# BUTSpeechFIT/huggingface_asr

Hardware: AMD Instinct MI355X
Metric: audio-seconds/sec encoder fwd+CTC, E-Branchformer-base (higher is better)
Workload: dtype bf16; 1 GPU; E-Branchformer-base enc+CTC (relative-pos), 32x10s 16kHz clips/GPU: fbank+CMVN -> conv2d sub -> 16 layers -> CTC head -> CTC loss (the batch-independent projection of the relative-position table, 0.2 % of the FLOPs, is cached across steps); per_gpu_batch=32, frames=1000, encoder_frames=250, parallelism=replicas x1 (no exchange step), steps_in_flight=4, wide_tiles=True, hw_queues=4

## Files before the change

### huggingface_asr_amd/_lib.py

```python
from __future__ import annotations

import ctypes as C
import os

_HERE = os.path.dirname(os.path.abspath(__file__))
LIB_PATH = os.environ.get("HFASR_HIP_LIB") or os.path.join(_HERE, "libhfasr_hip.so")

vp, i32, i64, f32, f64, sz = C.c_void_p, C.c_int, C.c_long, C.c_float, C.c_double, C.c_size_t


class EbfConfig(C.Structure):
    _fields_ = [(n, i32) for n in ("B", "T", "F", "d", "H", "I", "L", "V", "C1", "C2", "K", "stride", "pad",
                                   "is_causal", "pos_type", "csgu_kernel", "merge_kernel", "csgu_act", "use_macaron")] + \
               [("ln_eps", f32), ("logits_f32", i32), ("logits_ld", i32), ("branch_overlap", i32), ("extra_layers", i32), ("layer_mixing", i32), ("csgu_linear", i32),
                ("context_mode", i32), ("gate_blk", i32), ("ln_fold", i32), ("wide_tiles", i32)]


class LnRedDesc(C.Structure):
    _fields_ = [("partial", vp), ("nblk", i32), ("d", i32), ("dgamma", vp), ("dbeta", vp), ("kind", i32)]


class Gpt2Config(C.Structure):
    _fields_ = [("d", i32), ("H", i32), ("L", i32), ("V", i32), ("eps", f32), ("step_form", i32), ("act", i32)]

# ... 20 lines not shown
    "mi_layernorm_chain": [vp, i64, vp, i32, vp, vp, f32, vp, i64, vp, vp, f32, vp, i64, vp, i64, vp, vp, vp, i64, i32, i32, vp],
    "mi_cast_f32_bf16": [vp, i64, vp, i64, i32, i32, vp],
    "mi_rotary_bf16": [vp, i64, vp, i64, vp, vp, i32, i32, i32, i32, vp],
    "mi_attention_bf16": [vp, i64, vp, i64, vp, i64, i32, vp, i64, vp, vp, vp, vp, i64, i32, i32, i32, i32, f32, i32, vp],
    "mi_attention_qkv_bf16": [vp, i64, vp, i64, vp, i64, vp, i64, vp, vp, vp, vp, i64, i32, i32, i32, i64, i32, i32, f32, i32, vp],
    "mi_attention_qkv_bf16_v": [vp, i64, vp, i64, vp, i64, vp, i64, vp, vp, vp, vp, i64, i32, i32, i32, i64, i32, i32, f32, i32, i32, vp],
    "mi_attention_x_lse_bf16": [vp, i64, vp, i64, vp, i64, vp, vp, i64, vp, i32, i32, i32, i32, i32, f32, i32, f32, C.c_uint, C.c_uint, vp],
    "mi_attention_x_bwd_probs": [vp, i64, vp, i64, vp, i64, vp, vp, i64, vp, i64, vp, vp, vp, i64, vp, i64, i32, i32, i32, i32, i32, f32, i32, f32, C.c_uint, C.c_uint, vp],
    "mi_attention_qkv_lse_bf16": [vp, i64, vp, i64, vp, i64, vp, i64, vp, vp, vp, vp, i64, vp, i32, i32, i32, i32, f32, i32, f32, C.c_uint, C.c_uint, vp],
    "mi_attention_qkv_bwd_probs": [vp, i64, vp, i64, vp, i64, vp, i64, vp, vp, vp, vp, i64, vp, i64, vp, vp, vp, i64, vp, i64, i32,
                                   vp, i64, vp, vp, vp, vp, i64, i32, i32, i32, i32, f32, i32, f32, C.c_uint, C.c_uint, i32, vp],
    "mi_attention_qkv_bwd_fused": [vp, vp, vp, i64, vp, vp, i64, vp, i64, vp, vp, vp, vp, i64, vp, sz, i32, i32, i32, i32, f32, vp],
    "mi_row_stats_bf16": [vp, i64, i32, f32, vp, i32, vp],
    "mi_csgu_bf16": [vp, i64, vp, vp, vp, vp, vp, vp, i64, i32, i32, i32, i32, i32, i32, i32, vp],
    "mi_dwconv_residual_bf16": [vp, i64, vp, vp, vp, i64, i32, i32, i32, i32, i32, vp],
    "mi_fbank_f64": [vp, i64, vp, i32, vp, vp, vp, vp, vp, vp, i32, i32, i32, f64, f64, vp],
    "mi_trim_zeros_pad_f32": [vp, i64, vp, i32, i32, i32, vp, i64, i32, vp, vp, vp, vp],
    "mi_cmvn_utterance": [vp, vp, i32, i32, i32, i32, i32, f32, vp],
    "mi_cmvn_global": [vp, i64, i32, vp, vp, vp],
    "mi_row_lse": [vp, i64, i32, i32, vp, i32, vp],
    "mi_gemm_lse_f32": [vp, i64, vp, i64, vp, vp, i64, vp, vp, i32, i32, i32, vp],
    "mi_gemm_lse_workspace_floats": [i32, i32],
    "mi_row_argmax": [vp, i64, i32, i32, vp, i32, vp],
    "mi_ctc_collapse": [vp, i32, i32, vp, i32, i64, vp, i32, vp, vp, vp],
    "mi_ctc_greedy": [vp, i64, i64, i32, i32, i32, i32, vp, i32, i64, vp, vp, i32, vp, vp, vp],
    "mi_ctc_beam_workspace_bytes": [i32, i32, i32],
    "mi_ctc_beam_cut": [vp, i64, i64, i32, i32, i32, i32, vp, i32, i32, vp, vp, vp, vp, vp],
    "mi_ctc_beam_walk": [vp, i64, i64, i32, i32, i32, i32, vp, i32, i64, i32, i32, i32, vp, vp, vp, vp, vp, sz, vp, i32, vp, vp, vp, vp],
    "mi_gemm_argmax_workspace_floats": [i32, i32],
    "mi_gemm_argmax_bf16": [vp, i64, vp, i64, vp, vp, vp, i32, i32, i32, vp],
# ... 167 lines not shown
```

### huggingface_asr_amd/csrc/encoder.hip

```cpp
#include "common.hpp"
#include <hip/hip_ext.h>
#include <stdio.h>
#include "../../include/hfasr_hip.h"

namespace {

enum G { G_CONV1_W, G_CONV1_B, G_CONV2_W, G_CONV2_B, G_FEOUT_W, G_FEOUT_B, G_FP_LN_G, G_FP_LN_B, G_FP_W, G_FP_B,
         G_ENC_LN_G, G_ENC_LN_B, G_HEAD_W, G_HEAD_B, G_MIX_W ,
         G_GATE1_W, G_GATE1_B, G_GATE2_W, G_GATE2_B  };
enum LS { FF1_LN_G, FF1_LN_B, FF1_W1, FF1_B1, FF1_W2, FF1_B2,
          ATT_LN_G, ATT_LN_B, ATT_WQK, ATT_BQK, ATT_WV, ATT_BV, ATT_WO, ATT_BO, ATT_WPOS, ATT_U, ATT_V,
          MLP_LN_G, MLP_LN_B, MLP_W1, MLP_B1, CSGU_LN_G, CSGU_LN_B, CSGU_W, CSGU_B, MLP_W2, MLP_B2,
          MRG_DW_W, MRG_DW_B, MRG_W, MRG_B, FIN_LN_G, FIN_LN_B,
          FF2_LN_G, FF2_LN_B, FF2_W1, FF2_B1, FF2_W2, FF2_B2, CSGU_LIN_W, CSGU_LIN_B,
          FF1_WF, FF1_SF, FF1_CF, QKV_WF, QKV_SF, QKV_CF, MLP_WF, MLP_SF, MLP_CF, FF2_WF, FF2_SF, FF2_CF };

struct Dims { int T1, F1, T2, F2, M, Tp, hd; };

int conv_out(int n, int k, int s, int pad_total) { return (n + pad_total - k) / s + 1; }

Dims dims(const mi_ebf_config& c) {
    Dims d;
    const int pt = c.is_causal ? 2 * c.pad : 2 * c.pad;
    d.T1 = conv_out(c.T, c.K, c.stride, pt); d.F1 = conv_out(c.F, c.K, c.stride, pt);
// ... 261 lines not shown
    if (!c.ln_fold) RUN(enter_layer(w.x, 0));
    if (c.layer_mixing) RUN(mi_softmax_vec_f32(Gf(G_MIX_W), c.L + 1, w.sw, st));
    const int P = 2 * T2 - 1;
    if (c.pos_type == 1 && compute_posp)
        for (int l = 0; l < Lt; ++l)
            RUN(mi_gemm_bf16(pos_table, d, Lw(l, ATT_WPOS), d, nullptr, 0, (bf16_t*)posp + (size_t)l * P * d, d, 0, nullptr, 0, 1.f, 0,
                             P, d, d, 0, 0, st));
    const float* rot_cos = (const float*)pos_table;
    const float* rot_sin = rot_cos ? rot_cos + (size_t)T2 * D.hd : nullptr;
    const float scale = 1.0f / sqrtf((float)D.hd);
    const int kc = c.csgu_kernel, km = c.merge_kernel;

    if (c.ln_fold) {
        if (c.pos_type == 2 || !c.use_macaron || c.extra_layers || c.layer_mixing || c.csgu_linear || (D.hd != 64 && D.hd != 128)) return MI_ERR_ARG;
        const int gv = c.wide_tiles ? 40 : 0;
        const int npg = c.wide_tiles ? d / 64 : d / 32;
        RUN(mi_layernorm_fold(w.x, d, mask_len, T2, nullptr, nullptr, 0.f, w.x, d, w.a0, d, w.lnst, M, d, st));
        int np = 1;
        for (int l = 0; l < c.L; ++l) {
            if (hidden_states && hipMemcpyAsync(hidden_states + (size_t)l * M * d, w.x, (size_t)M * d * sizeof(float), hipMemcpyDeviceToDevice, st) != hipSuccess)
                return MI_ERR_LAUNCH;
            RUN(mi_gemm_lnfold_bf16(w.a0, d, Lw(l, FF1_WF), d, Lf(l, FF1_SF), Lf(l, FF1_CF), w.lnst, np, leps, w.h, I, 1, M, I, d, st));
            RUN(mi_gemm_resid_stats_f32_v(w.h, I, Lw(l, FF1_W2), I, Lf(l, FF1_B2), w.x, d, w.x, d, 0.5f, w.a0, d, w.lnst, M, d, I, gv, st));
            np = npg;
            RUN(mi_gemm_lnfold_bf16(w.a0, d, Lw(l, QKV_WF), d, Lf(l, QKV_SF), Lf(l, QKV_CF), w.lnst, np, leps, w.qk, 3 * d, 0, M, 3 * d, d, st));
            RUN(mi_attention_qkv_bf16(w.qk, 3 * d, w.qk + d, 3 * d, w.qk + 2 * d, 3 * d,
                                      c.pos_type == 1 ? (const bf16_t*)posp + (size_t)l * P * d : nullptr, d,
                                      c.pos_type == 1 ? Lf(l, ATT_U) : nullptr, c.pos_type == 1 ? Lf(l, ATT_V) : nullptr,
                                      mask_len, w.ctx, d, c.B, T2, 0, 0, c.H, D.hd, scale, c.is_causal, st));
            RUN(mi_gemm_bf16_v(w.ctx, d, Lw(l, ATT_WO), d, Lf(l, ATT_BO), 1, w.cat, 2 * d, 0, nullptr, 0, 1.f, 0, M, d, d, 0, 0, gv, st));
            RUN(mi_gemm_lnfold_bf16(w.a0, d, Lw(l, MLP_WF), d, Lf(l, MLP_SF), Lf(l, MLP_CF), w.lnst, np, leps, w.h, I, 1, M, I, d, st));
            RUN(mi_row_stats_bf16(w.h + I / 2, I, I / 2, leps, w.stats, M, st));
            const int dil = c.is_causal ? (kc - 1) / 2 : 1;
            const int cpad = c.is_causal ? (kc - 1) * dil : (kc - 1) / 2;
            RUN(mi_csgu_bf16(w.h, I, w.stats, Lf(l, CSGU_LN_G), Lf(l, CSGU_LN_B), Lf(l, CSGU_W), Lf(l, CSGU_B), w.s, I / 2, c.B, T2, I / 2, kc, cpad, dil, c.csgu_act, st));
            RUN(mi_gemm_bf16_v(w.s, I / 2, Lw(l, MLP_W2), I / 2, Lf(l, MLP_B2), 1, w.cat + d, 2 * d, 0, nullptr, 0, 1.f, 0, M, d, I / 2, 0, 0, gv, st));
            RUN(mi_dwconv_residual_bf16(w.cat, 2 * d, Lf(l, MRG_DW_W), Lf(l, MRG_DW_B), w.m2, 2 * d, c.B, T2, 2 * d, km, (km - 1) / 2, st));
            RUN(mi_gemm_resid_stats_f32_v(w.m2, 2 * d, Lw(l, MRG_W), 2 * d, Lf(l, MRG_B), w.x, d, w.x, d, 1.0f, w.a0, d, w.lnst, M, d, 2 * d, gv, st));
            RUN(mi_gemm_lnfold_bf16(w.a0, d, Lw(l, FF2_WF), d, Lf(l, FF2_SF), Lf(l, FF2_CF), w.lnst, np, leps, w.h, I, 1, M, I, d, st));
            RUN(mi_gemm_bf16_v(w.h, I, Lw(l, FF2_W2), I, Lf(l, FF2_B2), 1, w.x, d, 1, w.x, d, 0.5f, 0, M, d, I, 0, 0, gv, st));
            if (l + 1 == c.L) {
                RUN(mi_layernorm_chain(w.x, d, nullptr, T2, Lf(l, FIN_LN_G), Lf(l, FIN_LN_B), leps, nullptr, 0,
                                       Gf(G_ENC_LN_G), Gf(G_ENC_LN_B), c.ln_eps, w.hid, d, last_hidden, d, nullptr, nullptr, nullptr, 0, M, d, st));
            } else {
                RUN(mi_layernorm_fold(w.x, d, nullptr, T2, Lf(l, FIN_LN_G), Lf(l, FIN_LN_B), leps, w.x, d, w.a0, d, w.lnst, M, d, st));
                np = 1;
            }
        }
    } else
    for (int l = 0; l < Lt; ++l) {
        if (hidden_states && l < c.L && hipMemcpyAsync(hidden_states + (size_t)l * M * d, w.x, (size_t)M * d * sizeof(float), hipMemcpyDeviceToDevice, st) != hipSuccess)
            return MI_ERR_LAUNCH;
// ... 144 lines not shown
```

### huggingface_asr_amd/csrc/gemm_8p.hip

```cpp
#include "gemm_args.hpp"
#include <type_traits>

#ifndef GEMM_FLOOR
#define GEMM_FLOOR 0
#endif
#ifndef GEMM128_LOADER
#define GEMM128_LOADER 0
#endif

namespace {

typedef __attribute__((address_space(1))) const void* gptr_t;
typedef __attribute__((address_space(3))) void* lptr_t;

constexpr int TB = 256, BK = 64;
constexpr int BUF = 65536, BOFF = 32768;

template <int N>
__device__ __forceinline__ void wait_vm() {
    if constexpr (N >= 0) asm volatile("s_waitcnt vmcnt(%0)" ::"n"(N) : "memory");
}
__device__ __forceinline__ void barrier() {
    __builtin_amdgcn_sched_barrier(0);
    asm volatile("s_barrier" ::: "memory");
    __builtin_amdgcn_sched_barrier(0);
}
__device__ __forceinline__ void wait_lds() {
    asm volatile("s_waitcnt lgkmcnt(0)" ::: "memory");
    __builtin_amdgcn_sched_barrier(0);
}

__device__ __attribute__((aligned(16))) uint4 g_zero_page8p = {0u, 0u, 0u, 0u};

struct Ctx {
    const char* A; const char* W;
    unsigned offA[2][2], offB[2][2];
    int cti[2][2], cfi[2][2];
    unsigned dA[2][2], dB[2][2];
    unsigned aRd[2], bRd[2];
};

template <bool CONV, int ACT, bool OUT32 = false, bool GATED = false, bool LNF = false, bool LSE = false, bool AMAX = false, int CE = 0>
__global__ __launch_bounds__(512, 2) void gemm8p_kernel(GemmArgs p) {
    extern __shared__ __attribute__((aligned(16))) char smem[];
    const int tid = threadIdx.x, lane = tid & 63;
    const int wave = __builtin_amdgcn_readfirstlane(tid >> 6);
    const int wr = wave >> 2, wc = wave & 3;

    const int ntm = (p.M + TB - 1) / TB, ntn = (p.N + TB - 1) / TB;
    const int nwg = ntm * ntn;
    int bid = blockIdx.x;
    {
        const int q = nwg >> 3, r = nwg & 7, xcd = bid & 7, idx = bid >> 3;
        bid = (xcd < r ? xcd * (q + 1) : r * (q + 1) + (xcd - r) * q) + idx;
    }
    const int m0 = (bid / ntn) * TB, n0 = (bid % ntn) * TB;

    Ctx c;
    c.A = reinterpret_cast<const char*>(p.A);
    c.W = reinterpret_cast<const char*>(p.W);
    {
        const int prow = lane >> 3, pc = lane & 7;
#pragma unroll
        for (int h = 0; h < 2; ++h)
#pragma unroll
            for (int e = 0; e < 2; ++e) {
                const int ra = wr * 128 + h * 64 + (2 * wc + e) * 8;
                const int rb = (wave >> 1) * 64 + h * 32 + (2 * (wave & 1) + e) * 8;
                const int lcA = pc ^ (((ra + prow) >> 1) & 7), lcB = pc ^ (((rb + prow) >> 1) & 7);
                if constexpr (CONV) {
                    const int m = min(m0 + ra + prow, p.M - 1);
// ... 151 lines not shown
    if (wr == 1) barrier();
    unsigned cb = 0;
    int kt = 0;
    for (; kt < nk - 2; ++kt) {
        tile(kt, cb, T{}, T{}, T{}, T{}, std::integral_constant<int, 8>{}, std::integral_constant<int, 8>{}, std::integral_constant<int, 8>{});
        cb ^= BUF;
    }
    tile(kt, cb, T{}, T{}, F{}, F{}, std::integral_constant<int, 8>{}, std::integral_constant<int, 8>{}, std::integral_constant<int, 4>{});
    cb ^= BUF;
    tile(kt + 1, cb, F{}, F{}, F{}, F{}, std::integral_constant<int, 2>{}, std::integral_constant<int, 0>{}, std::integral_constant<int, -1>{});
    if (wr == 0) barrier();

    char* reg = smem + wave * 16384;
    const int fr = lane & 15, fq = lane >> 4, swz = (fr >> 1) & 7;
    const int nb = n0 + wc * 64;
    if constexpr (OUT32) {
        const int n4 = (p.N + 3) & ~3;
        float* C = reinterpret_cast<float*>(p.C);
#pragma unroll
        for (int j = 0; j < 4; ++j) {
            const int n = nb + j * 16 + fq * 4;
            f32x4 bj = f32x4{0.f, 0.f, 0.f, 0.f};
            if (p.bias_mode == 1) {
#pragma unroll
                for (int e = 0; e < 4; ++e)
                    if (n + e < p.N) bj[e] = p.bias[n + e];
            }
#pragma unroll
            for (int i = 0; i < 8; ++i) acc[i][j] += bj;
        }
// ... 832 lines not shown
        if ((a.N % TB) != 0 || (a.ldc % 8) != 0) return false;
        if (a.bias_mode == 1 && ((uintptr_t)a.bias & 15)) return false;
    }
    if (a.gated && (!conv || a.out_f32 || a.act != 1)) return false;
    if (a.ln_stats) {
        if (conv || a.out_f32 || a.gated || a.act > 1 || a.bias_mode != 1 || !a.ln_colsum || ((uintptr_t)a.ln_colsum & 15) || ((uintptr_t)a.ln_stats & 15)) return false;
        if (!(a.ln_npart == 1 || (a.ln_npart >= 4 && a.ln_npart <= 16 && (a.ln_npart % 4) == 0))) return false;
    }
    if (a.act >= 3) {
        if (conv || a.out_f32 || a.gated || a.ln_stats || a.resid || a.col_T || a.act > 4 || (a.aux_kind != 1 && a.aux_kind != 2) || a.drop_p < 0.f || a.drop_p >= 1.f) return false;
        if (a.act == 3 && (!a.aux || ((uintptr_t)a.aux & 15) || (a.ldaux % 8))) return false;
        if (a.act == 4 && (!a.C2 || ((uintptr_t)a.C2 & 15) || (a.ldc2 % 8))) return false;
    } else if (a.C2 || a.stats_out) {
        if (!a.out_f32 || !a.resid || a.N > 1024 || (a.C2 && (((uintptr_t)a.C2 & 7) || (a.ldc2 % 4))) || ((uintptr_t)a.stats_out & 7)) return false;
    }
    if (a.lse_part && (conv || !a.out_f32 || a.resid || a.C2 || a.stats_out || a.act != 0 || ((uintptr_t)a.lse_part & 7) || (a.lse_ld % 2) || a.lse_ld < 8 * cdiv(a.N, TB))) return false;
    if (a.amax_part && (conv || !a.out_f32 || a.resid || a.C2 || a.stats_out || a.lse_part || a.act != 0 || ((uintptr_t)a.amax_part & 7) || (a.amax_ld % 2) || a.amax_ld < 8 * cdiv(a.N, TB))) return false;
    if (a.ce) {
        if (a.ce < 1 || a.ce > 2 || conv || !a.out_f32 || a.resid || a.C2 || a.stats_out || a.amax_part || a.act != 0 || !a.ce_labels) return false;
        if (a.ce == 1 && (!a.lse_part || !a.ce_target)) return false;
        if (a.ce == 2 && (a.lse_part || !a.C || !a.ce_lse || !a.ce_g || (a.ldc % 8) != 0 || a.ldc < a.N || a.ldc > (long)TB * cdiv(a.N, TB))) return false;
    }
    if ((long)a.N * a.ldw * 2 >= (1l << 32)) return false;
    if (conv) {
        if ((a.Cin % BK) != 0 || a.Fout <= 0 || a.Tout <= 0) return false;
        if ((long)cdiv(a.M, (long)a.Fout * a.Tout) * a.Tin * a.Fin * a.Cin * 2 >= (1l << 32)) return false;
    } else if ((a.lda % 8) || (long)a.M * a.lda * 2 >= (1l << 32)) return false;
    return true;
}

template <typename K>
static bool set_lds_attr(K kernel, int bytes) { return ensure_dynamic_lds_ptr(reinterpret_cast<const void*>(kernel), (size_t)bytes); }

int gemm_8p_launch(const GemmArgs& a, bool conv, hipStream_t stream) {
    using kern_t = void (*)(GemmArgs);
    static const kern_t kerns[2][3] = {{gemm8p_kernel<false, 0>, gemm8p_kernel<false, 1>, gemm8p_kernel<false, 2>},
                                       {gemm8p_kernel<true, 0>, gemm8p_kernel<true, 1>, gemm8p_kernel<true, 2>}};
    if (a.act >= 0 && a.act <= 2 && !set_lds_attr(kerns[conv ? 1 : 0][a.act], 2 * BUF)) return MI_ERR_LAUNCH;
    if (a.act < 0 || a.act > 4) return MI_ERR_ARG;
    const int grid = cdiv(a.M, TB) * cdiv(a.N, TB);
    if (a.act >= 3) {
        const bool attr_t = set_lds_attr(gemm8p_kernel<false, 3>, 2 * BUF) && set_lds_attr(gemm8p_kernel<false, 4>, 2 * BUF);
        (void)attr_t;
        if (a.act == 3) launch_dense(PF_8P, gemm8p_kernel<false, 3>, dim3(grid), dim3(512), (size_t)2 * BUF, stream, a);
        else launch_dense(PF_8P_GELU, gemm8p_kernel<false, 4>, dim3(grid), dim3(512), (size_t)2 * BUF, stream, a);
        return MI_OK;
    }
    if (a.out_f32 && a.ce) {
        const kern_t kc = a.ce == 1 ? gemm8p_kernel<false, 0, true, false, false, false, false, 1> : gemm8p_kernel<false, 0, true, false, false, false, false, 2>;
        if (!set_lds_attr(kc, 2 * BUF)) return MI_ERR_LAUNCH;
// ... 73 lines not shown
```

### huggingface_asr_amd/csrc/gemm_args.hpp

```cpp
#pragma once
#include "common.hpp"
#include <hip/hip_ext.h>

struct GemmArgs {
    const bf16_t* A; long lda;
    const bf16_t* W; long ldw;
    const float* bias; int bias_mode;
    void* C; long ldc; int out_f32;
    const float* resid; long ldr; float alpha;
    int act;
    int col_T, col_Tp;
    int M, N, K;
    int variant;
    int Tin, Fin, Cin, Tout, Fout, KW, stride, pad_t, pad_f;
    int stride_f;
    int gated;
    const float* ln_stats; int ln_npart; const float* ln_colsum; float ln_eps;
    bf16_t* C2; long ldc2; float* stats_out;
    const bf16_t* aux; long ldaux; int aux_kind; float drop_p; unsigned long long drop_key;
    float* lse_part; int lse_ld;
    float* amax_part; int amax_ld;
    int ce; const long* ce_labels; float* ce_target; const float* ce_lse; const float* ce_g;
};
constexpr int LN_STATS_STRIDE = 32;

bool gemm_glds_supported(const GemmArgs& a, bool conv);
int gemm_glds_launch(const GemmArgs& a, bool conv, hipStream_t stream);


bool gemm_8p_supported(const GemmArgs& a, bool conv);
int gemm_8p_launch(const GemmArgs& a, bool conv, hipStream_t stream);
bool gemm_8p128_supported(const GemmArgs& a);
int gemm_8p128_launch(const GemmArgs& a, int ring, hipStream_t stream);


extern "C" int mi_profile_take_events(hipEvent_t* start, hipEvent_t* stop, int family);
enum { PF_8P = 0, PF_8P_GELU = 1, PF_8P_CONV = 2, PF_8P_OUT32 = 3, PF_8P128 = 4, PF_GLDS = 5, PF_GENERIC = 6, PF_8P_AMAX = 7, PF_8P_CE = 8, PF_COUNT = 9 };
// ... 8 lines not shown
```

### huggingface_asr_amd/csrc/gemm_bf16.hip

```cpp
#include "gemm_args.hpp"

namespace {

constexpr int BM = 128, BN = 128, BK = 64;
constexpr int NT = 256;

__device__ __forceinline__ int swz(int row, int chunk) { return chunk ^ ((row >> 1) & 7); }

template <bool CONV>
__global__ __launch_bounds__(NT) void gemm_bf16_kernel(GemmArgs p) {
    extern __shared__ __attribute__((aligned(16))) char smem[];
    bf16_t* sA = reinterpret_cast<bf16_t*>(smem);
    bf16_t* sB = sA + 2 * BM * BK;

    const int tid = threadIdx.x;
    const int lane = tid & 63, wave = tid >> 6;
    const int wm = wave >> 1, wn = wave & 1;

    const int ntm = (p.M + BM - 1) / BM, ntn = (p.N + BN - 1) / BN;
    const int nwg = ntm * ntn;
    int bid = blockIdx.x;
    {
        const int q = nwg >> 3, r = nwg & 7, xcd = bid & 7, idx = bid >> 3;
        bid = (xcd < r ? xcd * (q + 1) : r * (q + 1) + (xcd - r) * q) + idx;
// ... 301 lines not shown
    GemmArgs a{};
    a.A = (const bf16_t*)A; a.lda = lda; a.W = (const bf16_t*)W; a.ldw = ldw; a.bias = bias; a.bias_mode = bias ? 1 : 0;
    a.C = C; a.ldc = ldc; a.out_f32 = 1; a.resid = resid; a.ldr = ldr; a.alpha = alpha; a.act = 0; a.M = M; a.N = N; a.K = K;
    a.C2 = (bf16_t*)C2; a.ldc2 = ldc2; a.stats_out = stats_out;
    if (!A || !W || !C || !resid || (variant != 0 && variant != 40 && variant != 42 && variant != 43)) return MI_ERR_ARG;
    const bool wide = variant == 40;
    if (wide ? !gemm_8p_supported(a, false) : !gemm_8p128_supported(a)) return MI_ERR_UNSUPPORTED;
    const int slot = mi_profile_hook_begin(stream, 2.0 * M * N * K);
    const int rc = wide ? gemm_8p_launch(a, false, stream) : gemm_8p128_launch(a, variant == 42 ? 3 : (variant == 43 ? 2 : 0), stream);
    if (slot >= 0) mi_profile_hook_end(slot, stream);
    if (rc != MI_OK) return rc;
    MI_CHECK_LAUNCH();
    return MI_OK;
}

namespace {
__global__ __launch_bounds__(256) void lse_merge_kernel(const float* __restrict__ part, int ld, int npair, float* __restrict__ lse, int M) {
    const int g = threadIdx.x & 15;
    const int row = blockIdx.x * 16 + (threadIdx.x >> 4);
    const float* pr = part + (long)min(row, M - 1) * ld;
    float mx = -INFINITY;
    for (int t = g; t < npair; t += 16) mx = fmaxf(mx, pr[2 * t]);
    mx = fmaxf(mx, dpp_f32<0xB1, 0xF>(mx, mx)); mx = fmaxf(mx, dpp_f32<0x4E, 0xF>(mx, mx));
    mx = fmaxf(mx, dpp_f32<0x141, 0xF>(mx, mx)); mx = fmaxf(mx, dpp_f32<0x140, 0xF>(mx, mx));
    float s = 0.f;
    for (int t = g; t < npair; t += 16) {
        const f32x2 q = *reinterpret_cast<const f32x2*>(pr + 2 * t);
        if (q.x > -INFINITY) s += q.y * __expf(q.x - mx);
    }
    s += dpp_f32<0xB1, 0xF>(0.f, s); s += dpp_f32<0x4E, 0xF>(0.f, s);
// ... 137 lines not shown
```

### huggingface_asr_amd/engine.py

```python
from __future__ import annotations

import ctypes as C
import os

import torch

from . import _lib, ops
from .packing import _enc_map, encoder_specs, mapped_fp32, packed, relative_position_table, rotary_tables
from .shapes import GATE_SHARE, context_mode

G = dict(CONV1_W=0, CONV1_B=1, CONV2_W=2, CONV2_B=3, FEOUT_W=4, FEOUT_B=5, FP_LN_G=6, FP_LN_B=7, FP_W=8, FP_B=9,
         ENC_LN_G=10, ENC_LN_B=11, HEAD_W=12, HEAD_B=13, MIX_W=14, GATE1_W=15, GATE1_B=16, GATE2_W=17, GATE2_B=18)
LS = {n: i for i, n in enumerate(
    ["FF1_LN_G", "FF1_LN_B", "FF1_W1", "FF1_B1", "FF1_W2", "FF1_B2",
     "ATT_LN_G", "ATT_LN_B", "ATT_WQK", "ATT_BQK", "ATT_WV", "ATT_BV", "ATT_WO", "ATT_BO", "ATT_WPOS", "ATT_U", "ATT_V",
     "MLP_LN_G", "MLP_LN_B", "MLP_W1", "MLP_B1", "CSGU_LN_G", "CSGU_LN_B", "CSGU_W", "CSGU_B", "MLP_W2", "MLP_B2",
     "MRG_DW_W", "MRG_DW_B", "MRG_W", "MRG_B", "FIN_LN_G", "FIN_LN_B",
     "FF2_LN_G", "FF2_LN_B", "FF2_W1", "FF2_B1", "FF2_W2", "FF2_B2", "CSGU_LIN_W", "CSGU_LIN_B",
     "FF1_WF", "FF1_SF", "FF1_CF", "QKV_WF", "QKV_SF", "QKV_CF", "MLP_WF", "MLP_SF", "MLP_CF", "FF2_WF", "FF2_SF", "FF2_CF"])}
SLOT_RENAME = {"att_wqkv": "ATT_WQK", "att_bqkv": "ATT_BQK"}
FOLDS = {"ff1_b1": ("FF1", "ff1_w1", "ff1_ln_g", "ff1_ln_b"), "att_bqkv": ("QKV", "att_wqkv", "att_ln_g", "att_ln_b"),
         "mlp_b1": ("MLP", "mlp_w1", "mlp_ln_g", "mlp_ln_b"), "ff2_b1": ("FF2", "ff2_w1", "ff2_ln_g", "ff2_ln_b")}
ACT = {"identity": 0, "gelu": 1, "relu": 2, "silu": 3, "swish": 3}
POS = {None: 0, "none": 0, "relative": 1, "rotary": 2}
# ... 155 lines not shown
            return self._pos[key]
        d, H = c["hidden_size"], c["num_attention_heads"]
        if ptype == "relative":
            t = relative_position_table(T2, d).to(self.device).to(torch.float32 if self.precision == "fp32" else torch.bfloat16).contiguous()
        elif ptype == "rotary":
            cos, sin = rotary_tables(T2, d // H, c.get("rotary_embedding_base", 10000))
            t = torch.cat([cos.reshape(-1), sin.reshape(-1)]).to(self.device).contiguous()
        else:
            t = None
        self._pos[key] = t
        return t

    def _config_struct(self, B, T, F, slot=0):
        c = self.cfg
        fold = int(self._use_fold(B, self.out_frames(T)))
        return _lib.EbfConfig(ln_fold=fold, wide_tiles=int(bool(self.wide_tiles) and bool(fold)), B=B, T=T, F=F, d=c["hidden_size"], H=c["num_attention_heads"], I=c["intermediate_size"],
                              L=c["num_hidden_layers"], V=c["vocab_size"], C1=c["conv_dim"][0], C2=c["conv_dim"][1],
                              K=c["conv_kernel"][0], stride=c["conv_stride"][0], pad=c["conv_padding"][0],
                              is_causal=int(c.get("is_causal", False)), pos_type=POS[c.get("position_embeddings_type", "relative")],
                              csgu_kernel=c.get("csgu_kernel_size", 31), merge_kernel=c.get("merge_conv_kernel", 31),
                              csgu_act=ACT[c.get("csgu_activation", "identity")], use_macaron=int(c.get("use_macaron_ff", True)),
                              ln_eps=float(c.get("layer_norm_eps", 1e-5)), logits_f32=int(self.logits_dtype == torch.float32),
                              logits_ld=(c["vocab_size"] + 1 + 7) // 8 * 8,
                              branch_overlap=int(self.branch_overlap and slot == 0), extra_layers=self.extra, layer_mixing=self.mix,
                              csgu_linear=int(bool(c.get("csgu_use_linear_after_conv", False))), context_mode=self.ctx_mode, gate_blk=self.gate_blk)

    def _workspace(self, cs, slot=0):
        key = (cs.B, cs.T, cs.F, cs.ln_fold, cs.wide_tiles)
        if self._ws.get("key") != key:
            self._ws = {"key": key}
        if slot not in self._ws:
# ... 121 lines not shown
```

### huggingface_asr_amd/ops.py

```python
from __future__ import annotations

import math

import torch

from . import _lib

BF16 = torch.bfloat16


def _p(t):
    return 0 if t is None else t.data_ptr()


_PINNED_STREAM = None


def _stream():
    return torch.cuda.current_stream().cuda_stream if _PINNED_STREAM is None else _PINNED_STREAM


class pinned_stream:

    def __enter__(self):
# ... 238 lines not shown
def gate_act_mul(r, g, act=0):
    M, Cc = g.shape
    out = torch.empty((M, Cc), device=g.device, dtype=BF16)
    rc = _lib.lib().mi_gate_act_mul_bf16(r.data_ptr(), r.stride(0), g.data_ptr(), g.stride(0), out.data_ptr(), out.stride(0), M, Cc, int(act), _stream())
    _lib.check(rc, "mi_gate_act_mul_bf16")
    return out


def dwconv_residual(m, w, bias, B, T, pad_left=None):
    M, Cc = m.shape
    K = w.shape[-1]
    out = torch.empty_like(m)
    rc = _lib.lib().mi_dwconv_residual_bf16(m.data_ptr(), m.stride(0), w.data_ptr(), _p(bias), out.data_ptr(), out.stride(0),
                                            B, T, Cc, K, (K - 1) // 2 if pad_left is None else int(pad_left), _stream())
    _lib.check(rc, "mi_dwconv_residual_bf16")
    return out


def gemm_lse(a, w, bias, out):
    _req(a, BF16); _req(w, BF16)
    M, K = a.shape
    N = w.shape[0]
    L = _lib.lib()
    lse = torch.empty((M,), device=a.device, dtype=torch.float32)
    ws = torch.empty((int(L.mi_gemm_lse_workspace_floats(M, N)),), device=a.device, dtype=torch.float32)
    rc = L.mi_gemm_lse_f32(a.data_ptr(), a.stride(0), w.data_ptr(), w.stride(0), _p(bias), out.data_ptr(), out.stride(0), lse.data_ptr(), ws.data_ptr(), M, N, K, _stream())
    if rc == _lib.ERR_UNSUPPORTED:
        gemm(a, w, bias, out=out)
        return row_lse(out[:, :N])
    _lib.check(rc, "mi_gemm_lse_f32")
# ... 260 lines not shown
```

### huggingface_asr_amd/pipeline.py

```python
from __future__ import annotations

import os

import torch

from .engine import EBranchformerEngine


def reserve_hw_queues(lanes: int) -> int:
    want = 8 if lanes > 3 else 4
    have = os.environ.get("GPU_MAX_HW_QUEUES")
    if have is None and want > 4:
        if torch.cuda.is_initialized():
            raise RuntimeError("reserve_hw_queues: the HIP runtime is already initialised; export GPU_MAX_HW_QUEUES=8 before starting the process")
        os.environ["GPU_MAX_HW_QUEUES"] = str(want)
        return want
    return int(have) if have is not None else 4


class ForwardPipeline:
    def __init__(self, cfg: dict, device, state_dict: dict, lanes: int = 2, wide_tiles: bool = False, precision: str = "bf16"):
        if lanes < 1:
            raise ValueError("lanes >= 1")
        if precision != "bf16":
            raise NotImplementedError(f"ForwardPipeline lanes run in precision='bf16' only, got {precision!r}")
        self.device = torch.device(device)
        if lanes > 3 and int(os.environ.get("GPU_MAX_HW_QUEUES", "4")) < 8:
            import warnings
            warnings.warn("ForwardPipeline: more than 3 lanes on the HIP runtime's default 4 hardware queues — two lanes will take turns on one queue (measured: 4.6 instead of "
                          "3.8 ms per step); call pipeline.reserve_hw_queues(lanes) before the first HIP call of the process, or export GPU_MAX_HW_QUEUES=8", RuntimeWarning)
        self.engines = []
        for i in range(lanes):
            e = EBranchformerEngine(cfg, self.device)
            e.wide_tiles = bool(wide_tiles)
            if i == 0:
                e.load_state_dict(state_dict)
            else:
                e.share_weights_from(self.engines[0])
            self.engines.append(e)
        self.streams = [torch.cuda.Stream(device=self.device) for _ in range(lanes)] if lanes > 1 else [None]
        self.events = [None] * lanes
        self._next = 0

    @property
    def lanes(self) -> int:
        return len(self.engines)

    def submit(self, fn):
        lane = self._next
# ... 14 lines not shown
```

### include/hfasr_hip.h

```cpp
#ifndef HFASR_HIP_H
#define HFASR_HIP_H
#include <stddef.h>
#include <stdint.h>

#ifdef __cplusplus
extern "C" {
#endif

typedef struct ihipStream_t* mi_stream_t;

const char* mi_last_error(void);

int mi_profile_create(int capacity);
void mi_profile_enable(int on);
void mi_profile_reset(void);
int mi_profile_count(void);
int mi_profile_summary(double* total_ms, double* total_flops);
int mi_profile_calibrate(mi_stream_t stream, int n, double* median_ms);
int mi_profile_summary_family(int family, double* total_ms, double* total_flops, int* launches);

int mi_gemm_bf16(const void* A, long lda, const void* W, long ldw, const float* bias, int bias_mode,
                 void* C, long ldc, int out_f32, const float* resid, long ldr, float alpha, int act,
                 int M, int N, int K, int col_T, int col_Tp, mi_stream_t stream);
int mi_gemm_bf16_v(const void* A, long lda, const void* W, long ldw, const float* bias, int bias_mode,
// ... 75 lines not shown
                               void* dq, void* dk, void* dv, long ldg, void* workspace, size_t ws_bytes,
                               int B, int T, int H, int hd, float scale, mi_stream_t stream);
int mi_attention_x_lse_bf16(const void* q, long ldq, const void* k, long ldk, const void* v, long ldv, const int* lengths, void* out, long ldo, float* lse,
                            int B, int Tq, int Tk, int H, int hd, float scale, int causal, float drop_p, unsigned seed, unsigned stream_id, mi_stream_t stream);
int mi_attention_x_bwd_probs(const void* q, long ldq, const void* k, long ldk, const void* v, long ldv, const int* lengths, const void* ctx, long ldo,
                             const void* dctx, long ldd, const float* lse, void* prob, void* ds, long ldsr, void* dq, long lddq,
                             int B, int Tq, int Tk, int H, int hd, float scale, int causal, float drop_p, unsigned seed, unsigned stream_id, mi_stream_t stream);

int mi_row_stats_bf16(const void* x, long ldx, int d, float eps, float* stats, int M, mi_stream_t stream);
int mi_csgu_bf16(const void* u, long ldu, const float* stats, const float* gamma, const float* beta,
                 const float* w, const float* bias, void* out, long ldo,
                 int B, int T, int C, int K, int pad_left, int dilation, int act, mi_stream_t stream);

int mi_dwconv_residual_bf16(const void* m, long ldm, const float* w, const float* bias, void* out, long ldo,
                            int B, int T, int C, int K, int pad_left, mi_stream_t stream);
int mi_csgu_conv_bf16(const void* u, long ldu, const float* stats, const float* gamma, const float* beta, const float* w, const float* bias,
                      void* out, long ldo, int B, int T, int C, int K, int pad_left, int dilation, mi_stream_t stream);
int mi_gate_act_mul_bf16(const void* r, long ldr, const void* g, long ldg, void* out, long ldo, long M, int C, int act, mi_stream_t stream);
int mi_gate_act_mul_bwd_bf16(const void* r, long ldr, const void* g, long ldg, const void* ds, long ldds, void* dr, long lddr, void* dg, long lddg,
                             long M, int C, int act, mi_stream_t stream);

int mi_fbank_f64(const float* wave, long ldw, const int* num_samples, int N, const double* window,
                 const double* twiddle, const double* mel_t, const int* mel_lo, const int* mel_hi,
                 float* out, int T_out, int B, int nmel, double mel_floor, double preemph, mi_stream_t stream);
int mi_trim_zeros_pad_f32(const float* wave, long ldw, const int* num_samples, int N, int B, int min_len, float* out, long ldo, int N_out,
                          int* first, int* valid, int* eff_len, mi_stream_t stream);
int mi_cmvn_utterance(float* x, const int* frames, int B, int T, int nmel, int norm_means, int norm_vars,
                      float pad, mi_stream_t stream);
int mi_cmvn_global(float* x, long total, int nmel, const float* means, const float* stds, mi_stream_t stream);

// ... 285 lines not shown
```

Measured before the change: 71050 audio-seconds/sec.

## Fuse merge depthwise conv and residual into output-projection GEMM epilogues

After: 70950 audio-seconds/sec. No clear change (-0.1%).

```diff
diff --git a/huggingface_asr_amd/_lib.py b/huggingface_asr_amd/_lib.py
--- a/huggingface_asr_amd/_lib.py
+++ b/huggingface_asr_amd/_lib.py
@@ -58,6 +58,7 @@
     "mi_row_stats_bf16": [vp, i64, i32, f32, vp, i32, vp],
     "mi_csgu_bf16": [vp, i64, vp, vp, vp, vp, vp, vp, i64, i32, i32, i32, i32, i32, i32, i32, vp],
     "mi_dwconv_residual_bf16": [vp, i64, vp, vp, vp, i64, i32, i32, i32, i32, i32, vp],
+    "mi_gemm_dwres_bf16": [vp, i64, vp, i64, vp, vp, vp, i32, i32, vp, i64, i32, i32, i32, i32, vp],
     "mi_fbank_f64": [vp, i64, vp, i32, vp, vp, vp, vp, vp, vp, i32, i32, i32, f64, f64, vp],
     "mi_trim_zeros_pad_f32": [vp, i64, vp, i32, i32, i32, vp, i64, i32, vp, vp, vp, vp],
     "mi_cmvn_utterance": [vp, vp, i32, i32, i32, i32, i32, f32, vp],
diff --git a/huggingface_asr_amd/csrc/encoder.hip b/huggingface_asr_amd/csrc/encoder.hip
--- a/huggingface_asr_amd/csrc/encoder.hip
+++ b/huggingface_asr_amd/csrc/encoder.hip
@@ -299,6 +299,7 @@
     if (c.ln_fold) {
         if (c.pos_type == 2 || !c.use_macaron || c.extra_layers || c.layer_mixing || c.csgu_linear || (D.hd != 64 && D.hd != 128)) return MI_ERR_ARG;
         const int gv = c.wide_tiles ? 40 : 0;
+        const bool dwres = c.wide_tiles == 1 && km == 31 && T2 <= 256 && c.B == cdiv(M, 256) && (d % 256) == 0;
         const int npg = c.wide_tiles ? d / 64 : d / 32;
         RUN(mi_layernorm_fold(w.x, d, mask_len, T2, nullptr, nullptr, 0.f, w.x, d, w.a0, d, w.lnst, M, d, st));
         int np = 1;
@@ -313,14 +314,19 @@
                                       c.pos_type == 1 ? (const bf16_t*)posp + (size_t)l * P * d : nullptr, d,
                                       c.pos_type == 1 ? Lf(l, ATT_U) : nullptr, c.pos_type == 1 ? Lf(l, ATT_V) : nullptr,
                                       mask_len, w.ctx, d, c.B, T2, 0, 0, c.H, D.hd, scale, c.is_causal, st));
-            RUN(mi_gemm_bf16_v(w.ctx, d, Lw(l, ATT_WO), d, Lf(l, ATT_BO), 1, w.cat, 2 * d, 0, nullptr, 0, 1.f, 0, M, d, d, 0, 0, gv, st));
+            if (dwres) RUN(mi_gemm_dwres_bf16(w.ctx, d, Lw(l, ATT_WO), d, Lf(l, ATT_BO), Lf(l, MRG_DW_W), Lf(l, MRG_DW_B), km, 0, w.m2, 2 * d, c.B, T2, d, d, st));
+            else RUN(mi_gemm_bf16_v(w.ctx, d, Lw(l, ATT_WO), d, Lf(l, ATT_BO), 1, w.cat, 2 * d, 0, nullptr, 0, 1.f, 0, M, d, d, 0, 0, gv, st));
             RUN(mi_gemm_lnfold_bf16(w.a0, d, Lw(l, MLP_WF), d, Lf(l, MLP_SF), Lf(l, MLP_CF), w.lnst, np, leps, w.h, I, 1, M, I, d, st));
             RUN(mi_row_stats_bf16(w.h + I / 2, I, I / 2, leps, w.stats, M, st));
             const int dil = c.is_causal ? (kc - 1) / 2 : 1;
             const int cpad = c.is_causal ? (kc - 1) * dil : (kc - 1) / 2;
             RUN(mi_csgu_bf16(w.h, I, w.stats, Lf(l, CSGU_LN_G), Lf(l, CSGU_LN_B), Lf(l, CSGU_W), Lf(l, CSGU_B), w.s, I / 2, c.B, T2, I / 2, kc, cpad, dil, c.csgu_act, st));
-            RUN(mi_gemm_bf16_v(w.s, I / 2, Lw(l, MLP_W2), I / 2, Lf(l, MLP_B2), 1, w.cat + d, 2 * d, 0, nullptr, 0, 1.f, 0, M, d, I / 2, 0, 0, gv, st));
-            RUN(mi_dwconv_residual_bf16(w.cat, 2 * d, Lf(l, MRG_DW_W), Lf(l, MRG_DW_B), w.m2, 2 * d, c.B, T2, 2 * d, km, (km - 1) / 2, st));
+            if (dwres) {
+                RUN(mi_gemm_dwres_bf16(w.s, I / 2, Lw(l, MLP_W2), I / 2, Lf(l, MLP_B2), Lf(l, MRG_DW_W), Lf(l, MRG_DW_B), km, d, w.m2, 2 * d, c.B, T2, d, I / 2, st));
+            } else {
+                RUN(mi_gemm_bf16_v(w.s, I / 2, Lw(l, MLP_W2), I / 2, Lf(l, MLP_B2), 1, w.cat + d, 2 * d, 0, nullptr, 0, 1.f, 0, M, d, I / 2, 0, 0, gv, st));
+                RUN(mi_dwconv_residual_bf16(w.cat, 2 * d, Lf(l, MRG_DW_W), Lf(l, MRG_DW_B), w.m2, 2 * d, c.B, T2, 2 * d, km, (km - 1) / 2, st));
+            }
             RUN(mi_gemm_resid_stats_f32_v(w.m2, 2 * d, Lw(l, MRG_W), 2 * d, Lf(l, MRG_B), w.x, d, w.x, d, 1.0f, w.a0, d, w.lnst, M, d, 2 * d, gv, st));
             RUN(mi_gemm_lnfold_bf16(w.a0, d, Lw(l, FF2_WF), d, Lf(l, FF2_SF), Lf(l, FF2_CF), w.lnst, np, leps, w.h, I, 1, M, I, d, st));
             RUN(mi_gemm_bf16_v(w.h, I, Lw(l, FF2_W2), I, Lf(l, FF2_B2), 1, w.x, d, 1, w.x, d, 0.5f, 0, M, d, I, 0, 0, gv, st));
diff --git a/huggingface_asr_amd/csrc/gemm_8p.hip b/huggingface_asr_amd/csrc/gemm_8p.hip
--- a/huggingface_asr_amd/csrc/gemm_8p.hip
+++ b/huggingface_asr_amd/csrc/gemm_8p.hip
@@ -15,6 +15,7 @@
 
 constexpr int TB = 256, BK = 64;
 constexpr int BUF = 65536, BOFF = 32768;
+constexpr int DWE_K = 31, DWE_HALO = (DWE_K - 1) / 2, DWE_LD = TB * 2 + 16, DWE_ROWS = TB + 2 * DWE_HALO, DWE_PER = 32;
 
 template <int N>
 __device__ __forceinline__ void wait_vm() {
@@ -40,21 +41,22 @@
     unsigned aRd[2], bRd[2];
 };
 
-template <bool CONV, int ACT, bool OUT32 = false, bool GATED = false, bool LNF = false, bool LSE = false, bool AMAX = false, int CE = 0>
+template <bool CONV, int ACT, bool OUT32 = false, bool GATED = false, bool LNF = false, bool LSE = false, bool AMAX = false, int CE = 0, bool DWRES = false>
 __global__ __launch_bounds__(512, 2) void gemm8p_kernel(GemmArgs p) {
     extern __shared__ __attribute__((aligned(16))) char smem[];
     const int tid = threadIdx.x, lane = tid & 63;
     const int wave = __builtin_amdgcn_readfirstlane(tid >> 6);
     const int wr = wave >> 2, wc = wave & 3;
 
-    const int ntm = (p.M + TB - 1) / TB, ntn = (p.N + TB - 1) / TB;
+    const int mstep = DWRES ? p.utt_rows : TB;
+    const int ntm = (p.M + mstep - 1) / mstep, ntn = (p.N + TB - 1) / TB;
     const int nwg = ntm * ntn;
     int bid = blockIdx.x;
     {
         const int q = nwg >> 3, r = nwg & 7, xcd = bid & 7, idx = bid >> 3;
         bid = (xcd < r ? xcd * (q + 1) : r * (q + 1) + (xcd - r) * q) + idx;
     }
-    const int m0 = (bid / ntn) * TB, n0 = (bid % ntn) * TB;
+    const int m0 = (bid / ntn) * mstep, n0 = (bid % ntn) * TB;
 
     Ctx c;
     c.A = reinterpret_cast<const char*>(p.A);
@@ -236,6 +238,65 @@
     char* reg = smem + wave * 16384;
     const int fr = lane & 15, fq = lane >> 4, swz = (fr >> 1) & 7;
     const int nb = n0 + wc * 64;
+    if constexpr (DWRES) {
+        const int T = p.utt_rows;
+        f32x4 b4[4];
+#pragma unroll
+        for (int j = 0; j < 4; ++j)
+            b4[j] = (p.bias_mode == 1) ? *reinterpret_cast<const f32x4*>(p.bias + nb + j * 16 + fq * 4) : f32x4{0.f, 0.f, 0.f, 0.f};
+#pragma unroll
+        for (int i = 0; i < 8; ++i) {
+            const int row = wr * 128 + i * 16 + fr;
+#pragma unroll
+            for (int j = 0; j < 4; ++j) {
+                const f32x4 v = acc[i][j] + b4[j];
+                bf16x4 o = {f2bf(v.x), f2bf(v.y), f2bf(v.z), f2bf(v.w)};
+                if (row >= T) o = bf16x4{f2bf(0.f), f2bf(0.f), f2bf(0.f), f2bf(0.f)};
+                *reinterpret_cast<bf16x4*>(smem + (DWE_HALO + row) * DWE_LD + (wc * 64 + j * 16 + fq * 4) * 2) = o;
+            }
+        }
+        for (int id = tid; id < 2 * DWE_HALO * (TB / 4); id += 512) {
+            const int r = id / (TB / 4), ch = id % (TB / 4);
+            *reinterpret_cast<uint2*>(smem + (r < DWE_HALO ? r : TB + r) * DWE_LD + ch * 8) = uint2{0u, 0u};
+        }
+        const int cl = ((wave & 1) * 64 + lane) * 2, qd = wave >> 1;
+        const int cg = p.dw_col0 + n0 + cl;
+        float w0[DWE_K], w1[DWE_K];
+        {
+            const f32x2* wp = reinterpret_cast<const f32x2*>(p.dw_w + (long)cg * DWE_K);
+#pragma unroll
+            for (int q = 0; q < DWE_K; ++q) {
+                const f32x2 wv = wp[q];
+                if (2 * q < DWE_K) w0[2 * q] = wv.x; else w1[2 * q - DWE_K] = wv.x;
+                if (2 * q + 1 < DWE_K) w0[2 * q + 1] = wv.y; else w1[2 * q + 1 - DWE_K] = wv.y;
+            }
+        }
+        const float bs0 = p.dw_b ? p.dw_b[cg] : 0.f, bs1 = p.dw_b ? p.dw_b[cg + 1] : 0.f;
+        asm volatile("s_waitcnt lgkmcnt(0)" ::: "memory");
+        barrier();
+        bf16_t* out = p.dw_out + (long)m0 * p.dw_ldo + cg;
+#pragma unroll 1
+        for (int ck = 0; ck < 64 / DWE_PER; ++ck) {
+            const int t0 = qd * 64 + ck * DWE_PER;
+            if (t0 >= T) break;
+            const char* src = smem + t0 * DWE_LD + cl * 2;
+            float x0[DWE_PER + DWE_K - 1], x1[DWE_PER + DWE_K - 1];
+#pragma unroll
+            for (int i = 0; i < DWE_PER + DWE_K - 1; ++i) {
+                const bf16x2 u = *reinterpret_cast<const bf16x2*>(src + i * DWE_LD);
+                x0[i] = bf2f(u.x); x1[i] = bf2f(u.y);
+            }
+#pragma unroll
+            for (int j = 0; j < DWE_PER; ++j) {
+                float a0 = bs0, a1 = bs1;
+#pragma unroll
+                for (int k = 0; k < DWE_K; ++k) { a0 = fmaf(w0[k], x0[j + k], a0); a1 = fmaf(w1[k], x1[j + k], a1); }
+                const float o0 = x0[j + DWE_HALO] + a0, o1 = x1[j + DWE_HALO] + a1;
+                if (t0 + j < T) *reinterpret_cast<bf16x2*>(out + (long)(t0 + j) * p.dw_ldo) = bf16x2{f2bf(o0), f2bf(o1)};
+            }
+        }
+        return;
+    }
     if constexpr (OUT32) {
         const int n4 = (p.N + 3) & ~3;
         float* C = reinterpret_cast<float*>(p.C);
@@ -1098,6 +1159,10 @@
     } else if (a.C2 || a.stats_out) {
         if (!a.out_f32 || !a.resid || a.N > 1024 || (a.C2 && (((uintptr_t)a.C2 & 7) || (a.ldc2 % 4))) || ((uintptr_t)a.stats_out & 7)) return false;
     }
+    if (a.utt_rows) {
+        if (conv || a.out_f32 || a.gated || a.ln_stats || a.act != 0 || a.resid || a.C2 || a.stats_out || a.utt_rows < 0 || a.utt_rows > TB || (a.M % a.utt_rows) != 0) return false;
+        if (!a.dw_w || !a.dw_out || ((uintptr_t)a.dw_w & 7) || a.dw_col0 < 0 || (a.dw_col0 % 2) || ((uintptr_t)a.dw_out & 3) || (a.dw_ldo % 2)) return false;
+    }
     if (a.lse_part && (conv || !a.out_f32 || a.resid || a.C2 || a.stats_out || a.act != 0 || ((uintptr_t)a.lse_part & 7) || (a.lse_ld % 2) || a.lse_ld < 8 * cdiv(a.N, TB))) return false;
     if (a.amax_part && (conv || !a.out_f32 || a.resid || a.C2 || a.stats_out || a.lse_part || a.act != 0 || ((uintptr_t)a.amax_part & 7) || (a.amax_ld % 2) || a.amax_ld < 8 * cdiv(a.N, TB))) return false;
     if (a.ce) {
@@ -1118,6 +1183,12 @@
 
 int gemm_8p_launch(const GemmArgs& a, bool conv, hipStream_t stream) {
     using kern_t = void (*)(GemmArgs);
+    if (a.utt_rows) {
+        const kern_t kd = gemm8p_kernel<false, 0, false, false, false, false, false, 0, true>;
+        if (!set_lds_attr(kd, DWE_ROWS * DWE_LD)) return MI_ERR_LAUNCH;
+        launch_dense(PF_8P, kd, dim3((a.M / a.utt_rows) * (a.N / TB)), dim3(512), (size_t)DWE_ROWS * DWE_LD, stream, a);
+        return MI_OK;
+    }
     static const kern_t kerns[2][3] = {{gemm8p_kernel<false, 0>, gemm8p_kernel<false, 1>, gemm8p_kernel<false, 2>},
                                        {gemm8p_kernel<true, 0>, gemm8p_kernel<true, 1>, gemm8p_kernel<true, 2>}};
     if (a.act >= 0 && a.act <= 2 && !set_lds_attr(kerns[conv ? 1 : 0][a.act], 2 * BUF)) return MI_ERR_LAUNCH;
diff --git a/huggingface_asr_amd/csrc/gemm_args.hpp b/huggingface_asr_amd/csrc/gemm_args.hpp
--- a/huggingface_asr_amd/csrc/gemm_args.hpp
+++ b/huggingface_asr_amd/csrc/gemm_args.hpp
@@ -21,6 +21,7 @@
     float* lse_part; int lse_ld;
     float* amax_part; int amax_ld;
     int ce; const long* ce_labels; float* ce_target; const float* ce_lse; const float* ce_g;
+    int utt_rows; const float* dw_w; const float* dw_b; int dw_col0; bf16_t* dw_out; long dw_ldo;
 };
 constexpr int LN_STATS_STRIDE = 32;
 
diff --git a/huggingface_asr_amd/csrc/gemm_bf16.hip b/huggingface_asr_amd/csrc/gemm_bf16.hip
--- a/huggingface_asr_amd/csrc/gemm_bf16.hip
+++ b/huggingface_asr_amd/csrc/gemm_bf16.hip
@@ -339,6 +339,24 @@
     return MI_OK;
 }
 
+extern "C" int mi_gemm_dwres_bf16(const void* A, long lda, const void* W, long ldw, const float* bias, const float* dw_w, const float* dw_b, int dw_K, int col0,
+                                  void* out, long ldo, int B, int T, int N, int K, hipStream_t stream) {
+    MI_ENTER();
+    if (!A || !W || !dw_w || !out || B <= 0 || T <= 0 || N <= 0 || K <= 0 || dw_K <= 0 || col0 < 0 || ldo < (long)col0 + N) return MI_ERR_ARG;
+    if (dw_K != 31 || T > 256 || (long)B * T >= (1l << 31)) return MI_ERR_UNSUPPORTED;
+    GemmArgs a{};
+    a.A = (const bf16_t*)A; a.lda = lda; a.W = (const bf16_t*)W; a.ldw = ldw; a.bias = bias; a.bias_mode = bias ? 1 : 0;
+    a.alpha = 1.f; a.M = B * T; a.N = N; a.K = K;
+    a.utt_rows = T; a.dw_w = dw_w; a.dw_b = dw_b; a.dw_col0 = col0; a.dw_out = (bf16_t*)out; a.dw_ldo = ldo;
+    if (!gemm_8p_supported(a, false)) return MI_ERR_UNSUPPORTED;
+    const int slot = mi_profile_hook_begin(stream, 2.0 * a.M * N * K);
+    const int rc = gemm_8p_launch(a, false, stream);
+    if (slot >= 0) mi_profile_hook_end(slot, stream);
+    if (rc != MI_OK) return rc;
+    MI_CHECK_LAUNCH();
+    return MI_OK;
+}
+
 namespace {
 __global__ __launch_bounds__(256) void lse_merge_kernel(const float* __restrict__ part, int ld, int npair, float* __restrict__ lse, int M) {
     const int g = threadIdx.x & 15;
diff --git a/huggingface_asr_amd/engine.py b/huggingface_asr_amd/engine.py
--- a/huggingface_asr_amd/engine.py
+++ b/huggingface_asr_amd/engine.py
@@ -193,7 +193,7 @@
     def _config_struct(self, B, T, F, slot=0):
         c = self.cfg
         fold = int(self._use_fold(B, self.out_frames(T)))
-        return _lib.EbfConfig(ln_fold=fold, wide_tiles=int(bool(self.wide_tiles) and bool(fold)), B=B, T=T, F=F, d=c["hidden_size"], H=c["num_attention_heads"], I=c["intermediate_size"],
+        return _lib.EbfConfig(ln_fold=fold, wide_tiles=(2 if self.wide_tiles == 2 else int(bool(self.wide_tiles))) if fold else 0, B=B, T=T, F=F, d=c["hidden_size"], H=c["num_attention_heads"], I=c["intermediate_size"],
                               L=c["num_hidden_layers"], V=c["vocab_size"], C1=c["conv_dim"][0], C2=c["conv_dim"][1],
                               K=c["conv_kernel"][0], stride=c["conv_stride"][0], pad=c["conv_padding"][0],
                               is_causal=int(c.get("is_causal", False)), pos_type=POS[c.get("position_embeddings_type", "relative")],
diff --git a/huggingface_asr_amd/ops.py b/huggingface_asr_amd/ops.py
--- a/huggingface_asr_amd/ops.py
+++ b/huggingface_asr_amd/ops.py
@@ -276,6 +276,23 @@
     rc = _lib.lib().mi_dwconv_residual_bf16(m.data_ptr(), m.stride(0), w.data_ptr(), _p(bias), out.data_ptr(), out.stride(0),
                                             B, T, Cc, K, (K - 1) // 2 if pad_left is None else int(pad_left), _stream())
     _lib.check(rc, "mi_dwconv_residual_bf16")
+    return out
+
+
+def gemm_dwres(a, w, bias, dw_w, dw_bias, col0, out, B, T):
+    _req(a, BF16); _req(w, BF16); _req(out, BF16)
+    M, K = a.shape
+    N = w.shape[0]
+    if M != B * T or out.shape[0] != M:
+        raise ValueError("gemm_dwres: a and out need B * T rows")
+    if col0 < 0 or col0 + N > dw_w.shape[0] or col0 + N > out.shape[1] or (dw_bias is not None and dw_bias.shape[0] != dw_w.shape[0]):
+        raise ValueError("gemm_dwres: columns col0 .. col0 + N lie outside the depthwise weight or the output")
+    _req(dw_w, torch.float32)
+    if not dw_w.is_contiguous():
+        raise ValueError("gemm_dwres: the depthwise weight must be contiguous (C, taps)")
+    rc = _lib.lib().mi_gemm_dwres_bf16(a.data_ptr(), a.stride(0), w.data_ptr(), w.stride(0), _p(bias), dw_w.data_ptr(), _p(dw_bias), dw_w.shape[-1], int(col0),
+                                       out.data_ptr(), out.stride(0), B, T, N, K, _stream())
+    _lib.check(rc, "mi_gemm_dwres_bf16")
     return out
 
 
diff --git a/huggingface_asr_amd/pipeline.py b/huggingface_asr_amd/pipeline.py
--- a/huggingface_asr_amd/pipeline.py
+++ b/huggingface_asr_amd/pipeline.py
@@ -32,7 +32,7 @@
         self.engines = []
         for i in range(lanes):
             e = EBranchformerEngine(cfg, self.device)
-            e.wide_tiles = bool(wide_tiles)
+            e.wide_tiles = 2 if wide_tiles == 2 else bool(wide_tiles)
             if i == 0:
                 e.load_state_dict(state_dict)
             else:
diff --git a/include/hfasr_hip.h b/include/hfasr_hip.h
--- a/include/hfasr_hip.h
+++ b/include/hfasr_hip.h
@@ -113,6 +113,8 @@
 
 int mi_dwconv_residual_bf16(const void* m, long ldm, const float* w, const float* bias, void* out, long ldo,
                             int B, int T, int C, int K, int pad_left, mi_stream_t stream);
+int mi_gemm_dwres_bf16(const void* A, long lda, const void* W, long ldw, const float* bias, const float* dw_w, const float* dw_b, int dw_K, int col0,
+                       void* out, long ldo, int B, int T, int N, int K, mi_stream_t stream);
 int mi_csgu_conv_bf16(const void* u, long ldu, const float* stats, const float* gamma, const float* beta, const float* w, const float* bias,
                       void* out, long ldo, int B, int T, int C, int K, int pad_left, int dilation, mi_stream_t stream);
 int mi_gate_act_mul_bf16(const void* r, long ldr, const void* g, long ldg, void* out, long ldo, long M, int C, int act, mi_stream_t stream);
```
